# abargum/RAVE

Measured on AMD Instinct MI355X. Metric: audio samples/sec/GPU (48 kHz v2 encode+decode); × real-time factor, higher is better.
Workload: dtype fp32 (per conv / fused unit the faster of exact-fp32 MFMA and fp32 on the bf16 matrix cores: operands split exactly into 3 bf16 parts (24 significand bits), 6 of the 9 cross products (the 3 dropped are each < 2^-25 |a b|), fp32 accumulate; edges exact-fp32 MFMA); 1 GPU; v2 non-causal encode+decode, 16 x 65536 samples per GPU (BASELINE configs[1]); global_batch=16, samples_per_clip=65536, parallelism=dp1 (batch shards, RCCL all-gather of latents)

## Files before the change

### include/rave_amd.h

```cpp
#ifndef RAVE_AMD_H
#define RAVE_AMD_H

#include <stddef.h>
#include <stdint.h>

#ifdef __cplusplus
extern "C" {
#endif

#define RAVE_ABI_VERSION 21
#define RAVE_SPLITK_TICKETS 4096
#define RAVE_SPLITK_STATUS_WORD (RAVE_SPLITK_TICKETS - 1)

enum {
    RAVE_OK = 0,
    RAVE_ERR_ARG = -1,
    RAVE_ERR_HIP = -2,
    RAVE_ERR_UNSUPPORTED = -3,
    RAVE_ERR_STATE = -4,
    RAVE_ERR_COOP = -5
};

enum { RAVE_ACT_NONE = 0, RAVE_ACT_LEAKY = 1, RAVE_ACT_SNAKE = 2 };

// ... 169 lines not shown
    int32_t batch, frames, n_band, noise_bands;
    int32_t target, _pad0;
    const float* amp; int64_t a_sb, a_sc;
    const float* u;   int64_t u_sb;
    const float* gy;  int64_t gy_sb, gy_sc;
    float* gamp;      int64_t ga_sb, ga_sc;
} rave_noise_backward_args;
int rave_noise_synth_backward(const rave_noise_backward_args* a, void* stream);

typedef struct rave_adain_args {
    int32_t batch, channels, t_len, mode;
    int32_t max_batch, row0;
    const float* x; int64_t x_sb, x_sc;
    float* y;       int64_t y_sb, y_sc;
    float* stats;
    float* counters;
    uint32_t* ticket;
} rave_adain_args;
int rave_adain(const rave_adain_args* a, void* stream);

typedef struct rave_adain_backward_args {
    int32_t batch, channels, t_len, mode;
    int32_t max_batch, row0;
    const float* gy; int64_t gy_sb, gy_sc;
    float* gx;       int64_t gx_sb, gx_sc;
    const float* stats;
    const float* counters;
} rave_adain_backward_args;
int rave_adain_backward(const rave_adain_backward_args* a, void* stream);

typedef struct rave_unit_args {
    int32_t channels, batch, t_len, dilation;
    int32_t pad_left, act;
    float leaky_slope; int32_t precision;
    const float* x; int64_t x_sb, x_sc;
    float* y;       int64_t y_sb, y_sc;
    const float* weight;
    const float* bias1; const float* bias2;
    const float* alpha0; const float* alpha2;
    float* workspace;
    uint32_t* status;
    int32_t x_len;
    int32_t res_shift;
    int32_t coop_rb;
    int32_t reserved0;
} rave_unit_args;
int64_t rave_unit_packed_size(int channels);
int rave_unit_pack_weight(const float* w1, const float* w2, int channels, float* packed);
int64_t rave_unit_split_packed_size(int channels);
int rave_unit_split_pack_weight(const float* w1, const float* w2, int channels, float* packed);
int rave_unit_ring_pack_weight(const float* w1, const float* w2, int channels, float* packed);
int64_t rave_unit_bf3_packed_size(int channels);
int rave_unit_bf3_pack_weight(const float* w1, const float* w2, int channels, float* packed);
int64_t rave_unit_workspace(const rave_unit_args* a);
int rave_residual_unit(const rave_unit_args* a, void* stream);
int rave_debug_coop(int64_t spin_limit, int force_giveup);

#define RAVE_STACK_UNITS 3
typedef struct rave_stack_args {
    int32_t channels, batch, t_len, act;
    float leaky_slope; int32_t precision;
    int32_t dilation[RAVE_STACK_UNITS], pad_left[RAVE_STACK_UNITS];
    const float* x; int64_t x_sb, x_sc;
    float* y;       int64_t y_sb, y_sc;
    const float* weight[RAVE_STACK_UNITS];
    const float* bias1[RAVE_STACK_UNITS];
    const float* bias2[RAVE_STACK_UNITS];
    const float* alpha0[RAVE_STACK_UNITS];
    const float* alpha2[RAVE_STACK_UNITS];
} rave_stack_args;
int rave_stack_supported(int channels);
int rave_residual_stack(const rave_stack_args* a, void* stream);

typedef struct rave_edge_args {
    int32_t batch, frames;
    int32_t conv_c_in, conv_c_out, conv_kernel, conv_pad_left;
    int32_t pqmf_taps, pqmf_pad_left;
    int32_t mode, act;
    float leaky_slope;
    int32_t fill_channels, fill_t;
    int32_t precision;
    const float* x;     int64_t x_sb, x_sc;
    float* y;           int64_t y_sb, y_sc;
    const float* weight;
    const float* bias;
    const float* alpha;
    const float* filter;
    const float* noise; int64_t n_sb, n_sc;
    float* fill_y;      int64_t f_sb, f_sc;
    const float* fill_values;
    int64_t fill_vs;
} rave_edge_args;
int rave_encoder_head(const rave_edge_args* a, void* stream);
int rave_decoder_tail(const rave_edge_args* a, void* stream);
#define RAVE_EDGE_FILTER_FLOATS 8836
int rave_encoder_head_pack_filter(const float* hkf, int n_band, int taps, int n_out_bands, float* image);
int rave_decoder_tail_pack_filter(const float* hki, int n_band, int taps, float* image);
int rave_encoder_head_pack_filter_f32(const float* hkf, int n_band, int taps, int n_out_bands, float* image);
int rave_decoder_tail_pack_filter_f32(const float* hki, int n_band, int taps, float* image);

enum {
    RAVE_OP_CONV = 1,
    RAVE_OP_PQMF_ANALYSIS = 2,
    RAVE_OP_PQMF_SYNTHESIS = 3,
    RAVE_OP_FILL = 4,
    RAVE_OP_RVQ_ENCODE = 5,
// ... 265 lines not shown
```

### rave_amd/_native.py

```python
from __future__ import annotations

import ctypes as C
import os

_HERE = os.path.dirname(os.path.abspath(__file__))
LIB_PATH = os.path.join(_HERE, "librave_amd.so")
if os.environ.get("RAVE_AMD_DIAG_LIB") == "1":
    LIB_PATH = os.path.join(_HERE, "librave_amd_diag.so")
if os.environ.get("RAVE_AMD_LIB_VARIANT"):
    LIB_PATH = os.path.join(_HERE, f"librave_amd_{os.environ['RAVE_AMD_LIB_VARIANT']}.so")

RAVE_OK = 0
RAVE_ERR_ARG = -1
RAVE_ERR_HIP = -2
RAVE_ERR_UNSUPPORTED = -3
RAVE_ERR_STATE = -4
RAVE_ERR_COOP = -5

ACT = {"none": 0, "leaky": 1, "snake": 2}

OP_CONV = 1
OP_PQMF_ANALYSIS = 2
OP_PQMF_SYNTHESIS = 3
OP_FILL = 4
# ... 253 lines not shown
class ModelConfig(C.Structure):
    _fields_ = [("n_band", i32), ("enc_bands", i32), ("capacity", i32), ("latent_size", i32),
                ("kernel_size", i32), ("speaker_size", i32), ("n_ratios", i32),
                ("ratios", i32 * MAX_RATIOS), ("n_dilations", i32 * MAX_RATIOS),
                ("dilations", (i32 * MAX_DILATIONS) * MAX_RATIOS),
                ("amplitude_modulation", i32), ("causal", i32), ("activation", i32), ("adain", i32),
                ("leaky_slope", f32), ("conv_bias", i32), ("convt_bias", i32),
                ("noise", i32), ("noise_hidden", i32), ("noise_bands", i32), ("n_noise_ratios", i32),
                ("noise_ratios", i32 * MAX_RATIOS), ("rvq_quantizers", i32), ("rvq_codebook_size", i32),
                ("fuse_units", i32), ("speaker_rows", i32)]


class Param(C.Structure):
    _fields_ = [("name", C.c_char_p), ("data", vp), ("numel", i64)]


class OpInfo(C.Structure):
    _fields_ = [("kind", i32), ("precision", i32), ("flops", C.c_double), ("bytes", C.c_double),
                ("label", C.c_char * 96)]


PAYLOAD = 240


class PlanOp(C.Structure):
    _fields_ = [("kind", i32), ("_pad0", i32), ("raw", C.c_ubyte * PAYLOAD)]


class Reloc(C.Structure):
    _fields_ = [("op", i32), ("field_offset", i32), ("slot", i32), ("_pad0", i32),
                ("byte_offset", i64)]


STRUCTS = [ConvArgs, AnalysisArgs, SynthesisArgs, FillArgs, RvqArgs, ShiftArgs, PlanOp, Reloc,
           CopyArgs, NoiseArgs, AdainArgs, UnitArgs, StackArgs, ModelConfig, Param, OpInfo,
           FirArgs, RowStatsArgs, AttnPoolArgs, LinearArgs, MaxPoolArgs, EdgeArgs,
           StftArgs, DistanceArgs, YinArgs, F0OneHotArgs, SynthesisBackwardArgs, AnalysisBackwardArgs,
           ConvBackwardArgs, NoiseBackwardArgs, AdainBackwardArgs, StftLossArgs]

EXPORTS = [
    "rave_last_error", "rave_abi_version", "rave_struct_sizes",
    "rave_conv1d_chunk", "rave_conv1d_packed_size", "rave_conv1d_pack_weight", "rave_conv1d_pack_weight_device",
    "rave_conv1d",
    "rave_conv1d_workspace", "rave_conv1d_backward_workspace", "rave_conv1d_backward_data",
    "rave_conv1d_backward_weight", "rave_conv_transpose1d_backward_workspace", "rave_conv_transpose1d_backward_data",
    "rave_conv_transpose1d_backward_weight", "rave_conv1d_configs", "rave_conv1d_split_packed_size", "rave_conv1d_split_pack_weight",
    "rave_conv1d_ring_pack_weight", "rave_conv1d_bf3_packed_size", "rave_conv1d_bf3_pack_weight",
    "rave_pqmf_analysis", "rave_pqmf_synthesis", "rave_pqmf_analysis_backward", "rave_pqmf_synthesis_backward",
    "rave_fill_channels", "rave_copy",
    "rave_rvq_workspace", "rave_rvq_encode", "rave_rvq_decode", "rave_shift_history", "rave_noise_synth", "rave_adain",
    "rave_noise_synth_backward", "rave_adain_backward",
    "rave_unit_packed_size", "rave_unit_pack_weight", "rave_residual_unit",
    "rave_unit_split_packed_size", "rave_unit_split_pack_weight", "rave_unit_ring_pack_weight",
    "rave_unit_bf3_packed_size", "rave_unit_bf3_pack_weight",
    "rave_unit_workspace", "rave_debug_coop", "rave_model_check",
    "rave_stack_supported", "rave_residual_stack",
    "rave_plan_create", "rave_plan_run", "rave_plan_destroy", "rave_plan_size",
    "rave_plan_profile", "rave_plan_op_times", "rave_fill_uniform",
    "rave_model_param_count", "rave_model_param_info", "rave_model_create", "rave_model_destroy",
    "rave_model_encode", "rave_model_decode", "rave_model_forward", "rave_model_encode_codes",
    "rave_model_decode_codes", "rave_model_noise_shape", "rave_model_adain_control", "rave_model_set_row0",
    "rave_model_set_speaker", "rave_model_set_speakers", "rave_model_set_speaker_row0", "rave_model_speaker_info",
    "rave_model_adain_count", "rave_model_adain_info", "rave_model_adain_get", "rave_model_adain_set",
    "rave_model_tuning_get", "rave_model_tuning_set", "rave_model_plan_ops", "rave_model_profile",
    "rave_model_op_times", "rave_stream_create", "rave_stream_destroy", "rave_stream_reset",
    "rave_stream_encode", "rave_stream_decode", "rave_stream_encode_codes", "rave_stream_decode_codes",
    "rave_stream_delay",
    "rave_stream_launches",
    "rave_fir", "rave_row_stats", "rave_attn_pool", "rave_linear", "rave_maxpool",
    "rave_encoder_head", "rave_decoder_tail", "rave_encoder_head_pack_filter", "rave_decoder_tail_pack_filter",
    "rave_encoder_head_pack_filter_f32", "rave_decoder_tail_pack_filter_f32",
    "rave_stft_table_size", "rave_stft_pack_table", "rave_stft_mag",
    "rave_audio_distance_workspace", "rave_audio_distance",
    "rave_yin_shape", "rave_yin", "rave_f0_onehot", "rave_pitch_onehot",
    "rave_stft_loss_table_size", "rave_stft_loss_pack_table", "rave_stft_loss_workspace",
    "rave_stft_loss_forward", "rave_stft_loss_backward",
]
EDGE_FILTER_FLOATS = 8836


class NativeError(RuntimeError):
    pass


def _load():
    if not os.path.exists(LIB_PATH):
        raise ImportError(f"rave_amd native library not built: {LIB_PATH} is missing "
                          "(run `python -c 'import __graft_entry__ as g; g.build()'` or "
                          "`make -C rave_amd/csrc`)")
    lib = C.CDLL(LIB_PATH)
    lib.rave_last_error.restype = C.c_char_p
    lib.rave_abi_version.restype = C.c_int
    lib.rave_struct_sizes.argtypes = [C.POINTER(i64), C.c_int]
    lib.rave_conv1d_chunk.argtypes = [C.c_int] * 5
    lib.rave_conv1d_packed_size.argtypes = [C.c_int] * 6
    lib.rave_conv1d_packed_size.restype = i64
    lib.rave_conv1d_pack_weight.argtypes = [vp] + [C.c_int] * 7 + [vp]
    lib.rave_conv1d_pack_weight_device.argtypes = [vp] + [C.c_int] * 7 + [vp, vp]
    lib.rave_conv1d_workspace.argtypes = [C.POINTER(ConvArgs)]
    lib.rave_conv1d_configs.argtypes = [C.POINTER(ConvArgs), C.POINTER(i32), C.c_int]
    lib.rave_conv1d_split_packed_size.argtypes = [C.c_int] * 6
    lib.rave_conv1d_split_packed_size.restype = i64
    lib.rave_conv1d_split_pack_weight.argtypes = [vp] + [C.c_int] * 7 + [vp]
    lib.rave_conv1d_ring_pack_weight.argtypes = [vp] + [C.c_int] * 7 + [vp]
    lib.rave_conv1d_bf3_packed_size.argtypes = [C.c_int] * 6
    lib.rave_conv1d_bf3_packed_size.restype = i64
    lib.rave_conv1d_bf3_pack_weight.argtypes = [vp] + [C.c_int] * 7 + [vp]
    lib.rave_encoder_head_pack_filter.argtypes = [vp, C.c_int, C.c_int, C.c_int, vp]
    lib.rave_encoder_head_pack_filter_f32.argtypes = [vp, C.c_int, C.c_int, C.c_int, vp]
    lib.rave_decoder_tail_pack_filter_f32.argtypes = [vp, C.c_int, C.c_int, vp]
    lib.rave_decoder_tail_pack_filter.argtypes = [vp, C.c_int, C.c_int, vp]
    lib.rave_unit_packed_size.argtypes = [C.c_int]
    lib.rave_unit_packed_size.restype = i64
    lib.rave_unit_pack_weight.argtypes = [vp, vp, C.c_int, vp]
    lib.rave_unit_workspace.argtypes = [C.c_void_p]
    lib.rave_unit_workspace.restype = i64
    lib.rave_debug_coop.argtypes = [i64, C.c_int]
    lib.rave_unit_split_packed_size.argtypes = [C.c_int]
    lib.rave_stack_supported.argtypes = [C.c_int]
    lib.rave_unit_split_packed_size.restype = i64
    lib.rave_unit_split_pack_weight.argtypes = [vp, vp, C.c_int, vp]
    lib.rave_unit_ring_pack_weight.argtypes = [vp, vp, C.c_int, vp]
    lib.rave_unit_bf3_packed_size.argtypes = [C.c_int]
    lib.rave_unit_bf3_packed_size.restype = i64
    lib.rave_unit_bf3_pack_weight.argtypes = [vp, vp, C.c_int, vp]
    lib.rave_conv1d_workspace.restype = i64
    lib.rave_conv1d_backward_workspace.argtypes = [C.POINTER(ConvBackwardArgs)]
    lib.rave_conv1d_backward_workspace.restype = i64
    lib.rave_conv_transpose1d_backward_workspace.argtypes = [C.POINTER(ConvBackwardArgs)]
    lib.rave_conv_transpose1d_backward_workspace.restype = i64
    lib.rave_rvq_workspace.argtypes = [C.POINTER(RvqArgs)]
    lib.rave_rvq_workspace.restype = i64
    for name, st in [("rave_conv1d", ConvArgs), ("rave_pqmf_analysis", AnalysisArgs),
                     ("rave_pqmf_synthesis", SynthesisArgs), ("rave_fill_channels", FillArgs),
                     ("rave_pqmf_synthesis_backward", SynthesisBackwardArgs),
                     ("rave_pqmf_analysis_backward", AnalysisBackwardArgs),
                     ("rave_conv1d_backward_data", ConvBackwardArgs),
                     ("rave_conv1d_backward_weight", ConvBackwardArgs),
                     ("rave_conv_transpose1d_backward_data", ConvBackwardArgs),
                     ("rave_conv_transpose1d_backward_weight", ConvBackwardArgs),
                     ("rave_rvq_encode", RvqArgs), ("rave_rvq_decode", RvqArgs),
                     ("rave_shift_history", ShiftArgs), ("rave_copy", CopyArgs),
                     ("rave_noise_synth", NoiseArgs), ("rave_adain", AdainArgs),
                     ("rave_noise_synth_backward", NoiseBackwardArgs), ("rave_adain_backward", AdainBackwardArgs),
                     ("rave_residual_unit", UnitArgs), ("rave_residual_stack", StackArgs),
                     ("rave_fir", FirArgs), ("rave_row_stats", RowStatsArgs), ("rave_attn_pool", AttnPoolArgs),
                     ("rave_linear", LinearArgs), ("rave_maxpool", MaxPoolArgs),
                     ("rave_encoder_head", EdgeArgs), ("rave_decoder_tail", EdgeArgs)]:
        getattr(lib, name).argtypes = [C.POINTER(st), vp]
    lib.rave_stft_table_size.argtypes = [C.c_int]
    lib.rave_stft_table_size.restype = i64
    lib.rave_stft_pack_table.argtypes = [C.c_int, vp]
    lib.rave_stft_mag.argtypes = [C.POINTER(StftArgs), vp]
    lib.rave_audio_distance_workspace.argtypes = [C.POINTER(DistanceArgs)]
    lib.rave_audio_distance_workspace.restype = i64
    lib.rave_audio_distance.argtypes = [C.POINTER(DistanceArgs), vp]
    lib.rave_stft_loss_table_size.argtypes = [C.c_int, C.c_int]
    lib.rave_stft_loss_table_size.restype = i64
    lib.rave_stft_loss_pack_table.argtypes = [C.c_int, C.c_int, vp]
    lib.rave_stft_loss_workspace.argtypes = [C.POINTER(StftLossArgs)]
    lib.rave_stft_loss_workspace.restype = i64
    lib.rave_stft_loss_forward.argtypes = [C.POINTER(StftLossArgs), vp]
    lib.rave_stft_loss_backward.argtypes = [C.POINTER(StftLossArgs), vp]
    lib.rave_yin_shape.argtypes = [C.POINTER(YinArgs), C.POINTER(i32)]
    lib.rave_yin.argtypes = [C.POINTER(YinArgs), vp]
    lib.rave_f0_onehot.argtypes = [C.POINTER(F0OneHotArgs), vp]
    lib.rave_pitch_onehot.argtypes = [C.POINTER(YinArgs), C.POINTER(F0OneHotArgs), vp]
    lib.rave_plan_create.argtypes = [C.POINTER(PlanOp), C.c_int, C.POINTER(Reloc), C.c_int,
                                     C.POINTER(vp)]
    lib.rave_plan_run.argtypes = [vp, C.POINTER(vp), C.c_int, vp]
    lib.rave_plan_destroy.argtypes = [vp]
    lib.rave_plan_size.argtypes = [vp]
    lib.rave_plan_profile.argtypes = [vp, C.c_int]
    lib.rave_plan_op_times.argtypes = [vp, C.POINTER(C.c_float), C.c_int]
    lib.rave_fill_uniform.argtypes = [vp, i64, C.c_uint64, f32, f32, vp]
    cfgp = C.POINTER(ModelConfig)
    lib.rave_model_param_count.argtypes = [cfgp]
    lib.rave_model_param_info.argtypes = [cfgp, C.c_int, C.c_char_p, C.c_int, C.POINTER(i64)]
# ... 205 lines not shown
```

### rave_amd/csrc/unit_split.hip

```cpp
#include "common.h"
#include "pack_shared.h"

#include <algorithm>
#include <atomic>
#include <cmath>
#include <cstdlib>
#include <cstring>
#include <vector>

namespace rave {

typedef _Float16 us_h8 __attribute__((ext_vector_type(8)));
typedef _Float16 us_h4 __attribute__((ext_vector_type(4)));
typedef float us_f32x8 __attribute__((ext_vector_type(8)));
typedef float us_f32x4 __attribute__((ext_vector_type(4)));
typedef float us_f32x16 __attribute__((ext_vector_type(16)));
typedef unsigned us_u32x4 __attribute__((ext_vector_type(4)));
typedef __bf16 us_b8 __attribute__((ext_vector_type(8)));
typedef __bf16 us_b4 __attribute__((ext_vector_type(4)));

constexpr int kUSMaxDil = 16;
#ifndef RAVE_US_R
#define RAVE_US_R 3
#endif
// ... 13 lines not shown
#define US_AT(k, kc)                               \
    do {                                           \
        if ((k) >= 0) RAVE_STAMP(g_us_stamps, k); \
    } while (0)
#endif
constexpr unsigned kUSOOB = 0xFFFFFFF0u;
constexpr int kXcds = 8;
constexpr int kCoopNoFit = 1;
constexpr int kCoopMaxRB = 4;

struct USArgs {
    const float* x; float* y; const float* w; const float* rs1; const float* rs2;
    const float* b1; const float* b2; const float* a0; const float* a2;
    int64_t x_sb, x_sc, y_sb, y_sc;
    int T, d, pad_l, ntiles, XW;
    int XL, rsh;
    int x_bytes, y_bytes, w_bytes, bias_bytes;
    int act;
    float slope;
    unsigned xw_magic;
    unsigned* flags; unsigned* tmo; float* xmax; float* xch;
    int ngroups, xch_bytes;
    int xv;
    unsigned nb_magic;
    int flag_stride;
    unsigned* status;
    unsigned spin_limit;
    int force_giveup;
};

constexpr int kUSBf512Dil = 4;
template <int C, int WGN, int MI, int KG = 1, int CB = 2, int RB = 1, int NP = 2> struct USGeo {
    static constexpr int WGM = C / (32 * MI * RB), NWT = WGM * WGN, NW = NWT * KG, NT = 64 * NW;
    static constexpr int BN = 32 * CB * WGN;
    static constexpr int S1 = 3 * C / 16, S2 = C / 16, ST = S1 + S2;
    static constexpr int PH = C + 8;
    static constexpr int XW_MAX = BN + 2 * ((NP == 3 && C == 512) ? kUSBf512Dil : kUSMaxDil);
    static constexpr int XPLANE = XW_MAX * PH * 2;
    static constexpr int HPLANE = BN * PH * 2;
    static constexpr int PL1 = XPLANE > HPLANE ? XPLANE : HPLANE;
    static constexpr int PLANES = NP * PL1;
    static constexpr int TAB = PLANES, VOTE = PLANES + 6 * C * 4, VRED = VOTE + 16;
    static constexpr int LDS = VRED + 64;
    static constexpr int G8 = C / 8;
    static constexpr int XT = (XW_MAX * G8 + NT - 1) / NT;
    static constexpr int R = RB > 1 ? RAVE_US_RC : RAVE_US_R;
    static constexpr int G8R = C / (8 * RB);
    static constexpr int RED = NWT * MI * CB * 16 * 64 * 4;
    static_assert(C % 64 == 0 && (MI == 1 || MI == 2) && NW <= 16, "geometry");
    static_assert(RB == 1 || (KG == 1 && WGN == 1 && C % (32 * MI * RB) == 0), "cooperative geometry");
    static_assert(KG == 1 || (KG == 2 && S1 % 2 == 0 && S2 % 2 == 0 && RED <= PLANES), "K-groups");
};

template <int C, int WGN, int MI, int KG, int CB, bool SNAKE, int AR, int RB, bool GUARD>
__device__ __forceinline__ bool unit_split_body(const USArgs& a) {
    constexpr bool F32 = AR == 1, BF = AR == 2;
    constexpr int NPW = BF ? 3 : 2;
    using G = USGeo<C, WGN, MI, KG, CB, RB, NPW>;
    constexpr bool SC1X = RB > 1 && 2 * G::LDS > 160 * 1024;
    static_assert(!SC1X || 2 * G::LDS > 160 * 1024, "sc1 hand-off: one workgroup per CU only");
    constexpr bool GV = GUARD && AR == 0;
    static_assert(RB == 1 || GUARD || AR != 0, "the cooperative split16 form runs guarded");
    constexpr int NT = G::NT, PH = G::PH, G8 = G::G8, XT = G::XT, R = G::R;
    constexpr int S1 = G::S1, ST = G::ST, CG = C / 16;
    extern __shared__ __attribute__((aligned(16))) char lds[];
    _Float16* ph = reinterpret_cast<_Float16*>(lds);
    _Float16* pl = reinterpret_cast<_Float16*>(lds + G::PL1);
    _Float16* pm = reinterpret_cast<_Float16*>(lds + 2 * G::PL1);
    float* pf = reinterpret_cast<float*>(lds);
    float* tab = reinterpret_cast<float*>(lds + G::TAB);
    unsigned char* vote = reinterpret_cast<unsigned char*>(lds + G::VOTE);
    float* vred = reinterpret_cast<float*>(lds + G::VRED);

    US_AT(0, 0);
    const int tid = threadIdx.x;
    const int lane = tid & 63;
    const int wave = __builtin_amdgcn_readfirstlane(tid >> 6);
    const int kg = wave / G::NWT;
    const int twave = wave - kg * G::NWT;
    const int wm = twave % G::WGM, wn = twave / G::WGM;
    const int hh = lane >> 5, l32 = lane & 31;
    int lg, rb = 0;
    if constexpr (RB == 1) {
        lg = __builtin_amdgcn_readfirstlane(xcd_major(blockIdx.x, gridDim.x));
    } else {
        const int q = blockIdx.x >> 3;
        rb = q % RB;
        lg = (blockIdx.x & 7) * (int)(gridDim.x / (8 * RB)) + q / RB;
        if (lg >= a.ngroups) return true;
    }
    const int b = lg / a.ntiles;
    const int n0 = (lg - b * a.ntiles) * G::BN;
    const float slope = a.act == RAVE_ACT_LEAKY ? a.slope : 1.0f;
    const int XW = a.XW;
    const int ntask = XW * G8;
    const int t0 = n0 - a.pad_l;

    const auto xrs = make_rsrc(a.x + (int64_t)b * a.x_sb, a.x_bytes);
    const auto wrs = make_rsrc(a.w, a.w_bytes);
    int sh0 = 0, sh2 = 0;

    us_h8 ring[R][MI][NPW];
    const int wmg = wm + rb * G::WGM;
    const unsigned abase = (unsigned)((MI * wmg) * ST * NPW) * 1024u + (unsigned)lane * 16u;
    auto load_a = [&](int slot, int s) __attribute__((always_inline)) {
#pragma unroll
        for (int i = 0; i < MI; ++i)
#pragma unroll
            for (int p = 0; p < NPW; ++p)
                ring[slot][i][p] = __builtin_bit_cast(us_h8, __builtin_amdgcn_raw_buffer_load_b128(
                    wrs, s < ST ? abase + (unsigned)(((i * ST + s) * NPW + p) * 1024) : kUSOOB, 0, 0));
    };
    auto prefetch_ring = [&]() __attribute__((always_inline)) {
#pragma unroll
        for (int t = 0; t < R; ++t) load_a(t, t * KG + kg);
    };
    if (!a.xv) prefetch_ring();

    constexpr int NTAB = (6 * C + NT - 1) / NT;
    float tabv[NTAB];
#pragma unroll
    for (int r = 0; r < NTAB; ++r) {
        const int i = tid + r * NT;
        const int k = __builtin_amdgcn_readfirstlane(i / C), m = i - k * C;
        const float* src = k == 0 ? a.rs1 : k == 1 ? a.b1 : k == 2 ? a.a2 : k == 3 ? a.rs2 : k == 4 ? a.b2 : a.a0;
        const bool has = k < 6 && ((k == 1 || k == 4) ? a.bias_bytes > 0 : (k == 2 || k == 5) ? SNAKE : true);
        tabv[r] = has ? src[m] : 0.f;
    }
    auto store_tab = [&]() __attribute__((always_inline)) {
#pragma unroll
        for (int r = 0; r < NTAB; ++r)
            if (__builtin_amdgcn_readfirstlane(tid + r * NT) < 6 * C) tab[tid + r * NT] = tabv[r];
    };

    auto stage_window = [&](float xs) __attribute__((always_inline)) {
        float cmax = 0.f;
        float rx[XT][8];
#pragma unroll
        for (int i = 0; i < XT; ++i) {
            const int e = tid + i * NT;
            const int g = (int)(((unsigned)e * a.xw_magic) >> 24);
            const int w = e - g * XW;
            const int t = min(max(t0 + w, 0), a.XL - 1);
#pragma unroll
            for (int v = 0; v < 8; ++v) {
                const int c = min(g * 8 + v, C - 1);
                rx[i][v] = __builtin_bit_cast(float, __builtin_amdgcn_raw_buffer_load_b32(
                    xrs, (unsigned)(c * a.x_sc + t) * 4u, 0, 0));
            }
        }
#pragma unroll
        for (int i = 0; i < XT; ++i) {
            const int e = tid + i * NT;
            const int g = (int)(((unsigned)e * a.xw_magic) >> 24);
            const int w = e - g * XW;
            const bool ok = (e < ntask) && (t0 + w >= 0) && (t0 + w < a.XL);
            us_f32x8 v8;
#pragma unroll
            for (int v = 0; v < 8; ++v) {
                const float al = SNAKE ? a.a0[min(g * 8 + v, C - 1)] : 0.f;
                v8[v] = ok ? act<SNAKE>(rx[i][v], slope, al) * xs : 0.f;
            }
            if constexpr (F32) {
                if (e < ntask) {
                    *reinterpret_cast<us_f32x4*>(pf + w * PH + g * 8) = us_f32x4{v8[0], v8[1], v8[2], v8[3]};
                    *reinterpret_cast<us_f32x4*>(pf + w * PH + g * 8 + 4) = us_f32x4{v8[4], v8[5], v8[6], v8[7]};
                }
            } else if constexpr (BF) {
                us_b8 hi, mid, lo;
                bf3_split_pk(v8, hi, mid, lo);
// ... 28 lines not shown
            const int kb = e - g * nb;
            const int t = ta + 4 * kb;
            const bool ok = (e < ntv) && t >= 0 && t < a.XL;
#pragma unroll
            for (int v = 0; v < 8; ++v) {
                rx[i][v] = __builtin_bit_cast(us_f32x4, __builtin_amdgcn_raw_buffer_load_b128(
                    xrs, ok ? (unsigned)((g * 8 + v) * a.x_sc + t) * 4u : kUSOOB, 0, 0));
            }
        }
        prefetch_ring();
        if constexpr (SNAKE) {
            store_tab();
            __syncthreads();
        }
        if (RB == 1) US_AT(6, -1);
#pragma unroll
        for (int i = 0; i < XTV; ++i) {
            const int e = tid + i * NT;
            const int g = (int)(((unsigned)e * a.nb_magic) >> 24);
            const int kb = e - g * nb;
            if (e < ntv) {
                float al[8];
#pragma unroll
                for (int v = 0; v < 8; ++v) al[v] = SNAKE ? tab[5 * C + g * 8 + v] : 0.f;
#pragma unroll
                for (int q = 0; q < 4; ++q) {
                    const int w = ta + 4 * kb + q - t0;
                    us_f32x8 v8;
#pragma unroll
                    for (int v = 0; v < 8; ++v) v8[v] = act<SNAKE>(rx[i][v][q], slope, al[v]);
                    if (w < 0 || w >= XW) continue;
                    if constexpr (F32) {
                        *reinterpret_cast<us_f32x4*>(pf + w * PH + g * 8) = us_f32x4{v8[0], v8[1], v8[2], v8[3]};
                        *reinterpret_cast<us_f32x4*>(pf + w * PH + g * 8 + 4) = us_f32x4{v8[4], v8[5], v8[6], v8[7]};
                    } else if constexpr (BF) {
                        us_b8 hi, mid, lo;
                        bf3_split_pk(v8, hi, mid, lo);
                        *reinterpret_cast<us_b8*>(ph + w * PH + g * 8) = hi;
                        *reinterpret_cast<us_b8*>(pl + w * PH + g * 8) = lo;
                        *reinterpret_cast<us_b8*>(pm + w * PH + g * 8) = mid;
                    } else {
                        cmax = fmaxf(cmax, absmax8(v8));
                        const us_h8 hi = __builtin_convertvector(v8, us_h8);
                        const us_h8 lo = __builtin_convertvector((v8 - __builtin_convertvector(hi, us_f32x8)) * 2048.0f, us_h8);
                        *reinterpret_cast<us_h8*>(ph + w * PH + g * 8) = hi;
                        *reinterpret_cast<us_h8*>(pl + w * PH + g * 8) = lo;
                    }
                }
            }
        }
        if constexpr (!SNAKE) store_tab();
        return cmax;
    };
    {
        float cmax;
        if (a.xv) {
            cmax = stage_window_v();
        } else {
            store_tab();
            cmax = stage_window(1.0f);
        }
        if constexpr (GV) vote_cast(vote, wave, cmax);
        __syncthreads();
        if (GV && __builtin_expect(vote_any<G::NW>(vote), 0)) {
            sh0 = __builtin_amdgcn_readfirstlane(split_shift(block_max<G::NW>(cmax, vred)));
            const float xs = ldexpf(1.0f, -sh0);
#pragma nounroll
            for (int e = tid; e < ntask; e += NT) {
                const int g = (int)(((unsigned)e * a.xw_magic) >> 24);
                const int w = e - g * XW;
                const bool ok = (t0 + w >= 0) && (t0 + w < a.XL);
                const int t = min(max(t0 + w, 0), a.XL - 1);
                us_f32x8 v8;
#pragma unroll
                for (int v = 0; v < 8; ++v) {
                    const int c = min(g * 8 + v, C - 1);
                    const float xv = __builtin_bit_cast(float, __builtin_amdgcn_raw_buffer_load_b32(
                        xrs, (unsigned)(c * a.x_sc + t) * 4u, 0, 0));
                    v8[v] = ok ? act<SNAKE>(xv, slope, SNAKE ? a.a0[c] : 0.f) * xs : 0.f;
                }
                const us_h8 hi = __builtin_convertvector(v8, us_h8);
                const us_h8 lo = __builtin_convertvector((v8 - __builtin_convertvector(hi, us_f32x8)) * 2048.0f, us_h8);
                *reinterpret_cast<us_h8*>(ph + w * PH + g * 8) = hi;
                *reinterpret_cast<us_h8*>(pl + w * PH + g * 8) = lo;
            }
            __syncthreads();
        }
    }
    US_AT(1, 1);

    constexpr bool DA = RB > 1;
    us_f32x16 acc[MI][CB], accb[MI][CB];
    auto zero_acc = [&]() __attribute__((always_inline)) {
#pragma unroll
        for (int i = 0; i < MI; ++i)
#pragma unroll
            for (int j = 0; j < CB; ++j)
#pragma unroll
                for (int r = 0; r < 16; ++r) acc[i][j][r] = accb[i][j][r] = 0.f;
    };
    auto fold_acc = [&]() __attribute__((always_inline)) {
        if constexpr (DA) {
#pragma unroll
            for (int i = 0; i < MI; ++i)
#pragma unroll
                for (int j = 0; j < CB; ++j) acc[i][j] += accb[i][j];
        }
    };
    zero_acc();

    const int col0 = wn * 32 * CB + l32;
    struct BFr {
        us_h8 h[CB], l[CB], m[CB];
    };
    auto read_b = [&](int s, BFr& f) __attribute__((always_inline)) {
        int row, ch;
        if (s < S1) {
            const int tap = s / CG;
            row = col0 + tap * a.d;
            ch = (s - tap * CG) * 16;
        } else {
            row = col0;
            ch = (s - S1) * 16;
        }
#pragma unroll
        for (int j = 0; j < CB; ++j) {
            const int off = (row + j * 32) * PH + ch + 8 * hh;
            if constexpr (F32) {
                f.h[j] = *reinterpret_cast<const us_h8*>(pf + off);
                f.l[j] = *reinterpret_cast<const us_h8*>(pf + off + 4);
            } else {
                f.h[j] = *reinterpret_cast<const us_h8*>(ph + off);
                f.l[j] = *reinterpret_cast<const us_h8*>(pl + off);
                if constexpr (BF) f.m[j] = *reinterpret_cast<const us_h8*>(pm + off);
            }
        }
    };
    auto smap = [&](int t) __attribute__((always_inline)) {
        if (RB == 1 || t < S1 || t >= ST) return t;
        int u = t - S1 + rb * (CG / RB);
        if (u >= CG) u -= CG;
        return S1 + u;
    };
    auto step = [&](int t, int s, const BFr& f, us_f32x16 (&acc)[MI][CB]) __attribute__((always_inline)) {
        us_h8 ah[MI], al[MI], a2[MI];
#pragma unroll
        for (int i = 0; i < MI; ++i) {
            ah[i] = ring[t % R][i][0];
            al[i] = ring[t % R][i][1];
            a2[i] = ah[i] * (_Float16)2048.0f;
        }
        if constexpr (BF) {
            us_b8 wh[MI], wl[MI], wmd[MI];
#pragma unroll
            for (int i = 0; i < MI; ++i) {
                wh[i] = __builtin_bit_cast(us_b8, ring[t % R][i][0]);
                wl[i] = __builtin_bit_cast(us_b8, ring[t % R][i][1]);
                wmd[i] = __builtin_bit_cast(us_b8, ring[t % R][i][2]);
            }
            load_a(t % R, RB > 1 ? smap(t + R) : s + R * KG);
#pragma unroll
            for (int i = 0; i < MI; ++i)
#pragma unroll
                for (int j = 0; j < CB; ++j) {
                    const us_b8 xh = __builtin_bit_cast(us_b8, f.h[j]), xl = __builtin_bit_cast(us_b8, f.l[j]),
                                xm = __builtin_bit_cast(us_b8, f.m[j]);
                    acc[i][j] = __builtin_amdgcn_mfma_f32_32x32x16_bf16(wl[i], xh, acc[i][j], 0, 0, 0);
                    acc[i][j] = __builtin_amdgcn_mfma_f32_32x32x16_bf16(wh[i], xl, acc[i][j], 0, 0, 0);
                    acc[i][j] = __builtin_amdgcn_mfma_f32_32x32x16_bf16(wmd[i], xm, acc[i][j], 0, 0, 0);
                    acc[i][j] = __builtin_amdgcn_mfma_f32_32x32x16_bf16(wmd[i], xh, acc[i][j], 0, 0, 0);
                    acc[i][j] = __builtin_amdgcn_mfma_f32_32x32x16_bf16(wh[i], xm, acc[i][j], 0, 0, 0);
                    acc[i][j] = __builtin_amdgcn_mfma_f32_32x32x16_bf16(wh[i], xh, acc[i][j], 0, 0, 0);
                }
            return;
        }
        load_a(t % R, RB > 1 ? smap(t + R) : s + R * KG);
        if constexpr (F32) {
#pragma unroll
            for (int hf = 0; hf < 2; ++hf)
#pragma unroll
                for (int e = 0; e < 4; ++e)
#pragma unroll
                    for (int i = 0; i < MI; ++i)
#pragma unroll
                        for (int j = 0; j < CB; ++j) {
                            const us_f32x4 wv = __builtin_bit_cast(us_f32x4, hf ? al[i] : ah[i]);
                            const us_f32x4 xv = __builtin_bit_cast(us_f32x4, hf ? f.l[j] : f.h[j]);
                            acc[i][j] = __builtin_amdgcn_mfma_f32_32x32x2f32(wv[e], xv[e], acc[i][j], 0, 0, 0);
                        }
            return;
        }
#pragma unroll
        for (int i = 0; i < MI; ++i)
#pragma unroll
            for (int j = 0; j < CB; ++j) acc[i][j] = __builtin_amdgcn_mfma_f32_32x32x16_f16(a2[i], f.h[j], acc[i][j], 0, 0, 0);
#pragma unroll
        for (int i = 0; i < MI; ++i)
#pragma unroll
            for (int j = 0; j < CB; ++j) acc[i][j] = __builtin_amdgcn_mfma_f32_32x32x16_f16(ah[i], f.l[j], acc[i][j], 0, 0, 0);
#pragma unroll
        for (int i = 0; i < MI; ++i)
#pragma unroll
            for (int j = 0; j < CB; ++j) acc[i][j] = __builtin_amdgcn_mfma_f32_32x32x16_f16(al[i], f.h[j], acc[i][j], 0, 0, 0);
    };

    const int mrow0 = 32 * MI * wmg + 4 * hh;
    auto kloop = [&](auto gtag, auto t0tag, auto t1tag) __attribute__((always_inline)) {
        constexpr int GG = decltype(gtag)::value;
        constexpr int T0 = decltype(t0tag)::value, T1 = decltype(t1tag)::value;
        BFr f[2];
        auto sidx = [&](int t) __attribute__((always_inline)) { return RB > 1 ? smap(t) : t * KG + GG; };
        read_b(sidx(T0), f[0]);
#pragma unroll
        for (int t = T0; t < T1; ++t) {
            if (t + 1 < T1) read_b(sidx(t + 1), f[(t + 1 - T0) & 1]);
            __builtin_amdgcn_sched_barrier(0);
            if (DA && ((t - T0) & 1)) step(t, sidx(t), f[(t - T0) & 1], accb);
            else step(t, sidx(t), f[(t - T0) & 1], acc);
        }
    };
    float* red = reinterpret_cast<float*>(lds);
    auto combine = [&]() __attribute__((always_inline)) {
        if constexpr (KG == 2) {
            __syncthreads();
            float* mine = red + twave * (MI * CB * 16 * 64);
            if (kg == 1) {
#pragma unroll
                for (int i = 0; i < MI; ++i)
#pragma unroll
                    for (int j = 0; j < CB; ++j)
#pragma unroll
                        for (int r = 0; r < 16; ++r) mine[((i * CB + j) * 16 + r) * 64 + lane] = acc[i][j][r];
            }
            __syncthreads();
            if (kg == 0) {
#pragma unroll
                for (int i = 0; i < MI; ++i)
#pragma unroll
                    for (int j = 0; j < CB; ++j)
#pragma unroll
                        for (int r = 0; r < 16; ++r) acc[i][j][r] += mine[((i * CB + j) * 16 + r) * 64 + lane];
            }
        }
    };
    if (KG == 1 || kg == 0) kloop(IC<0>{}, IC<0>{}, IC<S1 / KG>{});
    else kloop(IC<1>{}, IC<0>{}, IC<S1 / KG>{});
    fold_acc();
    combine();
    __syncthreads();
    US_AT(2, 2);

    const float f0 = ldexpf(1.0f, sh0);
    const auto xcrs = make_rsrc(a.xch, RB > 1 ? a.xch_bytes : 0);
    const unsigned xslot = (unsigned)lg * (unsigned)(G::BN * C);
    auto seam = [&](float xs, auto pubtag) __attribute__((always_inline)) {
        constexpr bool publish = decltype(pubtag)::value != 0 && RB > 1;
        float cmax = 0.f;
        if (KG == 1 || kg == 0) {
#pragma unroll
            for (int i = 0; i < MI; ++i)
#pragma unroll
                for (int g = 0; g < 4; ++g) {
                    const int m = mrow0 + 32 * i + 8 * g;
                    const us_f32x4 rs = *reinterpret_cast<const us_f32x4*>(tab + m) * f0;
                    const us_f32x4 bb = *reinterpret_cast<const us_f32x4*>(tab + C + m);
                    us_f32x4 al = {0.f, 0.f, 0.f, 0.f};
                    if constexpr (SNAKE) al = *reinterpret_cast<const us_f32x4*>(tab + 2 * C + m);
#pragma unroll
                    for (int j = 0; j < CB; ++j) {
                        us_f32x4 v;
#pragma unroll
                        for (int e = 0; e < 4; ++e)
                            v[e] = act<SNAKE>(acc[i][j][4 * g + e] * rs[e] + bb[e], slope, al[e]) * xs;
                        if constexpr (publish)
                            __builtin_amdgcn_raw_buffer_store_b128(
                                __builtin_bit_cast(us_u32x4, v), xcrs,
                                (xslot + (unsigned)((col0 + 32 * j) * C + m)) * 4u, 0, 16);
                        if constexpr (F32) {
                            *reinterpret_cast<us_f32x4*>(pf + (col0 + 32 * j) * PH + m) = v;
                            continue;
                        }
                        if constexpr (BF) {
                            us_b4 hi, mid, lo;
                            bf3_split_pk(v, hi, mid, lo);
                            *reinterpret_cast<us_b4*>(ph + (col0 + 32 * j) * PH + m) = hi;
                            *reinterpret_cast<us_b4*>(pl + (col0 + 32 * j) * PH + m) = lo;
                            *reinterpret_cast<us_b4*>(pm + (col0 + 32 * j) * PH + m) = mid;
                            continue;
                        }
#pragma unroll
                        for (int e = 0; e < 4; ++e) cmax = fmaxf(cmax, fabsf(v[e]));
                        const us_h4 hv = __builtin_convertvector(v, us_h4);
                        const us_h4 lv = __builtin_convertvector((v - __builtin_convertvector(hv, us_f32x4)) * 2048.0f, us_h4);
                        *reinterpret_cast<us_h4*>(ph + (col0 + 32 * j) * PH + m) = hv;
                        *reinterpret_cast<us_h4*>(pl + (col0 + 32 * j) * PH + m) = lv;
                    }
                }
        }
        return cmax;
// ... 177 lines not shown
            const int n = n0 + col0 + 32 * j;
            const bool nok = n < a.T;
#pragma unroll
            for (int i = 0; i < MI; ++i)
#pragma unroll
                for (int r = 0; r < 16; ++r) {
                    const int m = mrow0 + 32 * i + 8 * (r >> 2) + (r & 3);
                    res[i][j][r] = __builtin_bit_cast(float, __builtin_amdgcn_raw_buffer_load_b32(
                        xrs, nok ? (unsigned)(m * a.x_sc + n + a.rsh) * 4u : kUSOOB, 0, 0));
                }
        }
#pragma unroll
        for (int i = 0; i < MI; ++i)
#pragma unroll
            for (int g = 0; g < 4; ++g) {
                const int m = mrow0 + 32 * i + 8 * g;
                const us_f32x4 rs = *reinterpret_cast<const us_f32x4*>(tab + 3 * C + m) * f2;
                const us_f32x4 bb = *reinterpret_cast<const us_f32x4*>(tab + 4 * C + m);
#pragma unroll
                for (int j = 0; j < CB; ++j) {
                    const int n = n0 + col0 + 32 * j;
                    const bool nok = n < a.T;
#pragma unroll
                    for (int e = 0; e < 4; ++e)
                        __builtin_amdgcn_raw_buffer_store_b32(
                            __builtin_bit_cast(unsigned, gave_up ? __builtin_nanf("")
                                                                 : acc[i][j][4 * g + e] * rs[e] + bb[e] + res[i][j][4 * g + e]),
                            yrs, nok ? (unsigned)((m + e) * a.y_sc + n) * 4u : kUSOOB, 0, 0);
                }
            }
    }
    US_AT(5, -1);
    if constexpr (CHECK && KG == 1) {
        if (vote_rerun()) return false;
    }
    return true;
}

template <int C, int WGN, int MI, int KG, int CB, bool SNAKE, int RB>
__global__ __launch_bounds__(64 * (C / (32 * MI * RB)) * WGN * KG) void unit_split_kernel(USArgs a) {
    if constexpr (RB > 1) {
        (void)unit_split_body<C, WGN, MI, KG, CB, SNAKE, 0, RB, true>(a);
    } else {
        if (!unit_split_body<C, WGN, MI, KG, CB, SNAKE, 0, RB, false>(a))
            (void)unit_split_body<C, WGN, MI, KG, CB, SNAKE, 0, RB, true>(a);
    }
}
template <int C, int WGN, int MI, int KG, int CB, bool SNAKE, int RB>
__global__ __launch_bounds__(64 * (C / (32 * MI * RB)) * WGN * KG) void unit_ring_f32_kernel(USArgs a) {
    (void)unit_split_body<C, WGN, MI, KG, CB, SNAKE, 1, RB, false>(a);
}
template <int C, int WGN, int MI, int KG, int CB, bool SNAKE, int RB>
__global__ __launch_bounds__(64 * (C / (32 * MI * RB)) * WGN * KG) void unit_bf3_kernel(USArgs a) {
    (void)unit_split_body<C, WGN, MI, KG, CB, SNAKE, 2, RB, false>(a);
}

static int coop_max_queues() {
    static const int q = [] {
        const char* e = std::getenv("GPU_MAX_HW_QUEUES");
        const int v = e ? std::atoi(e) : 0;
        return v > 0 ? v : 4;
    }();
    return q;
}

template <int C, int WGN, int MI, int KG, int CB, int RB = 1>
static int us_launch(USArgs k, int B, bool snake, int ar, hipStream_t st) {
    using G = USGeo<C, WGN, MI, KG, CB, RB>;
    using G3 = USGeo<C, WGN, MI, KG, CB, RB, 3>;
    const bool f32 = ar == 1;
    if (k.XW > (ar == 2 ? G3::XW_MAX : G::XW_MAX)) {
        set_error(ar == 2 && C == 512 ? "residual_unit(bf16x3): C = 512 supports dilations <= 4"
                                      : "residual_unit(split16): dilation too large");
        return RAVE_ERR_UNSUPPORTED;
    }
    k.ntiles = ceil_div(k.T, G::BN);
    void (*kern)(USArgs) = nullptr;
    int lds = G::LDS;
    if (ar == 2) {
        if constexpr (G3::LDS <= 160 * 1024) {
            kern = snake ? unit_bf3_kernel<C, WGN, MI, KG, CB, true, RB> : unit_bf3_kernel<C, WGN, MI, KG, CB, false, RB>;
            lds = G3::LDS;
        } else {
            set_error("residual_unit(bf16x3): this width does not fit the CU's LDS as three planes");
            return RAVE_ERR_UNSUPPORTED;
        }
    } else {
        kern = f32 ? (snake ? unit_ring_f32_kernel<C, WGN, MI, KG, CB, true, RB> : unit_ring_f32_kernel<C, WGN, MI, KG, CB, false, RB>)
                   : (snake ? unit_split_kernel<C, WGN, MI, KG, CB, true, RB> : unit_split_kernel<C, WGN, MI, KG, CB, false, RB>);
    }
    static bool attr[6] = {false, false, false, false, false, false};
    if (lds > 65536 && !attr[2 * ar + snake]) {
        RAVE_CHECK_HIP(hipFuncSetAttribute(reinterpret_cast<const void*>(kern),
                                           hipFuncAttributeMaxDynamicSharedMemorySize, lds));
        attr[2 * ar + snake] = true;
    }
    int grid = k.ntiles * B;
    if constexpr (RB > 1) {
        static int fits[6] = {-1, -1, -1, -1, -1, -1};
        int& f = fits[2 * ar + snake];
        if (f < 0) {
            int per_cu = 0, dev = 0, cus = 0;
            RAVE_CHECK_HIP(hipOccupancyMaxActiveBlocksPerMultiprocessor(&per_cu, reinterpret_cast<const void*>(kern),
                                                                        G::NT, lds));
            RAVE_CHECK_HIP(hipGetDevice(&dev));
            RAVE_CHECK_HIP(hipDeviceGetAttribute(&cus, hipDeviceAttributeMultiprocessorCount, dev));
            const int64_t q = coop_max_queues();
// ... 21 lines not shown
extern "C" int64_t rave_unit_split_packed_size(int C) { return unit_packed_floats(C, 2); }
extern "C" int64_t rave_unit_bf3_packed_size(int C) { return unit_packed_floats(C, 3); }

static int unit_pack(const float* w1, const float* w2, int C, float* packed, int mode) {
    const bool f32 = mode != kPackSplit16;
    RAVE_CHECK_ARG(w1 && w2 && packed, "unit_split_pack_weight: null pointer");
    if (!us_supported(C)) {
        set_error("unit_split_pack_weight: split16 fused residual unit supports C in {64, 128, 256, 512}");
        return RAVE_ERR_UNSUPPORTED;
    }
    const int S1 = 3 * C / 16, ST = 4 * C / 16, CG = C / 16;
    std::vector<int> e1(C), e2(C);
    for (int m = 0; m < C; ++m) {
        double a1 = 0.0, a2 = 0.0;
        for (int k = 0; k < 3 * C; ++k) a1 = std::max(a1, (double)std::fabs(w1[(int64_t)m * 3 * C + k]));
        for (int k = 0; k < C; ++k) a2 = std::max(a2, (double)std::fabs(w2[(int64_t)m * C + k]));
        e1[m] = f32 ? 0 : row_exponent(a1);
        e2[m] = f32 ? 0 : row_exponent(a2);
    }
    for (int mb = 0; mb < C / 32; ++mb)
        for (int s = 0; s < ST; ++s)
            for (int l = 0; l < 64; ++l)
                for (int e = 0; e < 8; ++e) {
                    const int m = mb * 32 + (l & 31);
                    const int kk = 8 * (l >> 5) + e;
                    float v;
                    if (s < S1) {
                        const int tap = s / CG, ci = (s % CG) * 16 + kk;
                        v = std::ldexp(w1[((int64_t)m * C + ci) * 3 + tap], e1[m]);
                    } else {
                        const int ci = (s - S1) * 16 + kk;
                        v = std::ldexp(w2[(int64_t)m * C + ci], e2[m]);
                    }
                    put_fragment(packed, (int64_t)mb * ST + s, mode, l, e, v);
                }
    float* rs = packed + packed_floats((int64_t)(C / 32) * ST, pack_planes(mode), 0);
    for (int m = 0; m < C; ++m) {
        rs[m] = f32 ? 1.0f : (float)std::ldexp(1.0, -(e1[m] + 11));
        rs[C + m] = f32 ? 1.0f : (float)std::ldexp(1.0, -(e2[m] + 11));
    }
    return RAVE_OK;
}

extern "C" int rave_unit_split_pack_weight(const float* w1, const float* w2, int C, float* packed) {
    return unit_pack(w1, w2, C, packed, kPackSplit16);
}

extern "C" int rave_unit_ring_pack_weight(const float* w1, const float* w2, int C, float* packed) {
    return unit_pack(w1, w2, C, packed, kPackF32);
}

extern "C" int rave_unit_bf3_pack_weight(const float* w1, const float* w2, int C, float* packed) {
    return unit_pack(w1, w2, C, packed, kPackBf16x3);
}

#ifdef RAVE_STAMPS
extern "C" int rave_diag_unit_stamps(void* p) {
    RAVE_CHECK_HIP(hipMemcpyToSymbol(HIP_SYMBOL(g_us_stamps), &p, sizeof(p)));
    return RAVE_OK;
}
#endif

namespace rave {
static std::atomic<unsigned> g_coop_spin{kUSSpinLimit};
static std::atomic<int> g_coop_force{0};
static bool coop_enabled() {
    static const bool on = [] {
        const char* e = std::getenv("RAVE_UNIT_COOP");
        return !(e && e[0] == '0');
    }();
    return on;
}
constexpr int kCoopBN = 32;
struct CoopLayout {
    int rb = 1, stride = 2;
    int64_t groups = 0, xmax = 0, xch = 0, floats = 0;
};
static CoopLayout coop_layout(const rave_unit_args& a) {
    CoopLayout L;
    const int C = a.channels;
    if ((C != 256 && C != 512) || !coop_enabled() || a.batch <= 0 || a.t_len <= 0) return L;
    if (a.precision != RAVE_PREC_SPLIT16 && a.precision != RAVE_PREC_F32_RING && a.precision != RAVE_PREC_BF16X3)
        return L;
    const int64_t ng = (int64_t)ceil_div(a.t_len, kCoopBN) * a.batch;
    const int64_t ngp = ceil_div64(ng, 8) * 8;
    if (2 * ngp > RAVE_SPLITK_STATUS_WORD) return L;
    while (L.stride < 32 && 2 * L.stride * ngp <= RAVE_SPLITK_STATUS_WORD) L.stride *= 2;
    const int rb = a.coop_rb == 4 && C == 256 ? 4 : C / 128;
    if (a.coop_rb != 0 && a.coop_rb != rb) return L;
    L.groups = ng;
    L.xmax = RAVE_SPLITK_TICKETS;
    L.xch = L.xmax + ceil_div64(ngp * rb, 64) * 64;
    L.floats = L.xch + ngp * kCoopBN * C;
    if (ngp * kCoopBN * C * 4 >= (1ll << 31)) return CoopLayout{};
    L.rb = rb;
    return L;
}

int residual_unit_split(const rave_unit_args& a, void* stream) {
    const int C = a.channels;
    if (!us_supported(C)) {
        set_error("residual_unit(split16): fused unit supports C in {64, 128, 256, 512}");
        return RAVE_ERR_UNSUPPORTED;
    }
    if (a.coop_rb != 0 && !((C == 256 && (a.coop_rb == 2 || a.coop_rb == 4)) || (C == 512 && a.coop_rb == 4))) {
        set_error("residual_unit: coop_rb must be 0, or 2 / 4 at C = 256, 4 at C = 512");
// ... 136 lines not shown
```

Before: 1.415 billion samples/s.

## Overlap bf16x3 window staging with first-conv MFMA steps via channel chunks

```diff
diff --git a/include/rave_amd.h b/include/rave_amd.h
--- a/include/rave_amd.h
+++ b/include/rave_amd.h
@@ -245,6 +245,7 @@
 int rave_unit_ring_pack_weight(const float* w1, const float* w2, int channels, float* packed);
 int64_t rave_unit_bf3_packed_size(int channels);
 int rave_unit_bf3_pack_weight(const float* w1, const float* w2, int channels, float* packed);
+int rave_unit_bf3_step_map(int channels, int coop_rb, int* steps, int cap);
 int64_t rave_unit_workspace(const rave_unit_args* a);
 int rave_residual_unit(const rave_unit_args* a, void* stream);
 int rave_debug_coop(int64_t spin_limit, int force_giveup);
diff --git a/rave_amd/_native.py b/rave_amd/_native.py
--- a/rave_amd/_native.py
+++ b/rave_amd/_native.py
@@ -329,7 +329,7 @@
     "rave_noise_synth_backward", "rave_adain_backward",
     "rave_unit_packed_size", "rave_unit_pack_weight", "rave_residual_unit",
     "rave_unit_split_packed_size", "rave_unit_split_pack_weight", "rave_unit_ring_pack_weight",
-    "rave_unit_bf3_packed_size", "rave_unit_bf3_pack_weight",
+    "rave_unit_bf3_packed_size", "rave_unit_bf3_pack_weight", "rave_unit_bf3_step_map",
     "rave_unit_workspace", "rave_debug_coop", "rave_model_check",
     "rave_stack_supported", "rave_residual_stack",
     "rave_plan_create", "rave_plan_run", "rave_plan_destroy", "rave_plan_size",
@@ -401,6 +401,7 @@
     lib.rave_unit_bf3_packed_size.argtypes = [C.c_int]
     lib.rave_unit_bf3_packed_size.restype = i64
     lib.rave_unit_bf3_pack_weight.argtypes = [vp, vp, C.c_int, vp]
+    lib.rave_unit_bf3_step_map.argtypes = [C.c_int, C.c_int, C.POINTER(i32), C.c_int]
     lib.rave_conv1d_workspace.restype = i64
     lib.rave_conv1d_backward_workspace.argtypes = [C.POINTER(ConvBackwardArgs)]
     lib.rave_conv1d_backward_workspace.restype = i64
diff --git a/rave_amd/csrc/unit_split.hip b/rave_amd/csrc/unit_split.hip
--- a/rave_amd/csrc/unit_split.hip
+++ b/rave_amd/csrc/unit_split.hip
@@ -89,9 +89,30 @@
     static_assert(KG == 1 || (KG == 2 && S1 % 2 == 0 && S2 % 2 == 0 && RED <= PLANES), "K-groups");
 };
 
-template <int C, int WGN, int MI, int KG, int CB, bool SNAKE, int AR, int RB, bool GUARD>
+constexpr int us_chunk_step(int C, int NCH, int t) {
+    const int CG = C / 16, CGC = CG / NCH, SC = 3 * CGC;
+    const int c = t / SC, u = t - c * SC, tap = u / CGC;
+    return tap * CG + c * CGC + (u - tap * CGC);
+}
+constexpr bool us_chunk_map_ok(int C, int NCH) {
+    const int CG = C / 16, S1 = 3 * CG;
+    if (NCH < 1 || CG % NCH != 0 || S1 > 96) return false;
+    bool seen[96] = {};
+    for (int t = 0; t < S1; ++t) {
+        const int s = us_chunk_step(C, NCH, t);
+        if (s < 0 || s >= S1 || seen[s]) return false;
+        seen[s] = true;
+        if ((s % CG) * 16 + 16 > (t / (S1 / NCH) + 1) * (C / NCH)) return false;
+    }
+    return true;
+}
+constexpr int us_bf3_chunks(int C, int RB) { return RB > 1 ? 2 : 1; }
+
+template <int C, int WGN, int MI, int KG, int CB, bool SNAKE, int AR, int RB, bool GUARD, int NCH = 1>
 __device__ __forceinline__ bool unit_split_body(const USArgs& a) {
     constexpr bool F32 = AR == 1, BF = AR == 2;
+    static_assert(NCH == 1 || (BF && us_chunk_map_ok(C, NCH) && (3 * C / 16) % (NCH * KG) == 0),
+                  "window chunks: bf16x3 only, whole 16-channel groups and K-group steps per chunk");
     constexpr int NPW = BF ? 3 : 2;
     using G = USGeo<C, WGN, MI, KG, CB, RB, NPW>;
     constexpr bool SC1X = RB > 1 && 2 * G::LDS > 160 * 1024;
@@ -152,7 +173,7 @@
 #pragma unroll
         for (int t = 0; t < R; ++t) load_a(t, t * KG + kg);
     };
-    if (!a.xv) prefetch_ring();
+    if (NCH == 1 && !a.xv) prefetch_ring();
 
     constexpr int NTAB = (6 * C + NT - 1) / NT;
     float tabv[NTAB];
@@ -287,7 +308,7 @@
         if constexpr (!SNAKE) store_tab();
         return cmax;
     };
-    {
+    if constexpr (NCH == 1) {
         float cmax;
         if (a.xv) {
             cmax = stage_window_v();
@@ -321,8 +342,8 @@
             }
             __syncthreads();
         }
-    }
-    US_AT(1, 1);
+        US_AT(1, 1);
+    }
 
     constexpr bool DA = RB > 1;
     us_f32x16 acc[MI][CB], accb[MI][CB];
@@ -372,12 +393,13 @@
         }
     };
     auto smap = [&](int t) __attribute__((always_inline)) {
+        if (NCH > 1 && t < S1) return us_chunk_step(C, NCH, t);
         if (RB == 1 || t < S1 || t >= ST) return t;
         int u = t - S1 + rb * (CG / RB);
         if (u >= CG) u -= CG;
         return S1 + u;
     };
-    auto step = [&](int t, int s, const BFr& f, us_f32x16 (&acc)[MI][CB]) __attribute__((always_inline)) {
+    auto step = [&](int t, int sn, const BFr& f, us_f32x16 (&acc)[MI][CB]) __attribute__((always_inline)) {
         us_h8 ah[MI], al[MI], a2[MI];
 #pragma unroll
         for (int i = 0; i < MI; ++i) {
@@ -393,7 +415,7 @@
                 wl[i] = __builtin_bit_cast(us_b8, ring[t % R][i][1]);
                 wmd[i] = __builtin_bit_cast(us_b8, ring[t % R][i][2]);
             }
-            load_a(t % R, RB > 1 ? smap(t + R) : s + R * KG);
+            load_a(t % R, sn);
 #pragma unroll
             for (int i = 0; i < MI; ++i)
 #pragma unroll
@@ -409,7 +431,7 @@
                 }
             return;
         }
-        load_a(t % R, RB > 1 ? smap(t + R) : s + R * KG);
+        load_a(t % R, sn);
         if constexpr (F32) {
 #pragma unroll
             for (int hf = 0; hf < 2; ++hf)
@@ -444,14 +466,14 @@
         constexpr int GG = decltype(gtag)::value;
         constexpr int T0 = decltype(t0tag)::value, T1 = decltype(t1tag)::value;
         BFr f[2];
-        auto sidx = [&](int t) __attribute__((always_inline)) { return RB > 1 ? smap(t) : t * KG + GG; };
+        auto sidx = [&](int t) __attribute__((always_inline)) { return smap(t * KG + GG); };
         read_b(sidx(T0), f[0]);
 #pragma unroll
         for (int t = T0; t < T1; ++t) {
             if (t + 1 < T1) read_b(sidx(t + 1), f[(t + 1 - T0) & 1]);
             __builtin_amdgcn_sched_barrier(0);
-            if (DA && ((t - T0) & 1)) step(t, sidx(t), f[(t - T0) & 1], accb);
-            else step(t, sidx(t), f[(t - T0) & 1], acc);
+            if (DA && ((t - T0) & 1)) step(t, sidx(t + R), f[(t - T0) & 1], accb);
+            else step(t, sidx(t + R), f[(t - T0) & 1], acc);
         }
     };
     float* red = reinterpret_cast<float*>(lds);
@@ -478,8 +500,112 @@
             }
         }
     };
-    if (KG == 1 || kg == 0) kloop(IC<0>{}, IC<0>{}, IC<S1 / KG>{});
-    else kloop(IC<1>{}, IC<0>{}, IC<S1 / KG>{});
+    auto phase1_chunked = [&](auto xvtag, auto gtag) __attribute__((always_inline)) {
+        constexpr bool XV = decltype(xvtag)::value != 0;
+        constexpr int GG = decltype(gtag)::value;
+        constexpr int G8C = G8 / NCH, SCL = S1 / (NCH * KG);
+        constexpr int NBM = (G::XW_MAX + 3) / 4 + 1;
+        constexpr int NTK = ((XV ? G8C * NBM : G8C * G::XW_MAX) + NT - 1) / NT;
+        constexpr int NU = XV ? 4 * NTK : NTK;
+        const int ta = t0 & ~3;
+        const int per = XV ? (t0 + XW - ta + 3) >> 2 : XW;
+        const unsigned magic = XV ? a.nb_magic : a.xw_magic;
+        const int ntc = G8C * per;
+        us_f32x4 rv[2][XV ? NTK : 1][8];
+        float rs[2][XV ? 1 : NTK][8];
+        auto sidx = [&](int t) __attribute__((always_inline)) { return smap(t * KG + GG); };
+        auto issue = [&](int c) __attribute__((always_inline)) {
+#pragma unroll
+            for (int i = 0; i < NTK; ++i) {
+                const int e = tid + i * NT;
+                const int gl = (int)(((unsigned)e * magic) >> 24);
+                const int k = e - gl * per;
+                const int g = c * G8C + gl;
+                if constexpr (XV) {
+                    const int t = ta + 4 * k;
+                    const bool ok = (e < ntc) && t >= 0 && t < a.XL;
+#pragma unroll
+                    for (int v = 0; v < 8; ++v)
+                        rv[c & 1][i][v] = __builtin_bit_cast(us_f32x4, __builtin_amdgcn_raw_buffer_load_b128(
+                            xrs, ok ? (unsigned)((g * 8 + v) * a.x_sc + t) * 4u : kUSOOB, 0, 0));
+                } else {
+                    const int t = min(max(t0 + k, 0), a.XL - 1);
+#pragma unroll
+                    for (int v = 0; v < 8; ++v)
+                        rs[c & 1][i][v] = __builtin_bit_cast(float, __builtin_amdgcn_raw_buffer_load_b32(
+                            xrs, (e < ntc) ? (unsigned)((g * 8 + v) * a.x_sc + t) * 4u : kUSOOB, 0, 0));
+                }
+            }
+        };
+        auto split_row = [&](int c, int u) __attribute__((always_inline)) {
+            const int i = XV ? u >> 2 : u, q = u & 3;
+            const int e = tid + i * NT;
+            const int gl = (int)(((unsigned)e * magic) >> 24);
+            const int k = e - gl * per;
+            const int g = c * G8C + gl;
+            const int w = XV ? ta + 4 * k + q - t0 : k;
+            const bool live = (e < ntc) && w >= 0 && w < XW;
+            const bool inx = XV || ((t0 + w >= 0) && (t0 + w < a.XL));
+            us_f32x8 v8;
+#pragma unroll
+            for (int v = 0; v < 8; ++v) {
+                const float al = SNAKE ? tab[5 * C + min(g, G8 - 1) * 8 + v] : 0.f;
+                const float xv = XV ? rv[c & 1][i][v][q] : rs[c & 1][i][v];
+                v8[v] = inx ? act<SNAKE>(xv, slope, al) : 0.f;
+            }
+            us_b8 hi, mid, lo;
+            bf3_split_pk(v8, hi, mid, lo);
+            if (live) {
+                *reinterpret_cast<us_b8*>(ph + w * PH + g * 8) = hi;
+                *reinterpret_cast<us_b8*>(pl + w * PH + g * 8) = lo;
+                *reinterpret_cast<us_b8*>(pm + w * PH + g * 8) = mid;
+            }
+        };
+        issue(0);
+#pragma unroll
+        for (int t = 0; t < R; ++t) load_a(t, sidx(t));
+        issue(1);
+        store_tab();
+        if constexpr (SNAKE) __syncthreads();
+        if (RB == 1) US_AT(6, -1);
+#pragma unroll
+        for (int u = 0; u < NU; ++u) split_row(0, u);
+        __syncthreads();
+        US_AT(1, 1);
+#pragma unroll
+        for (int c = 0; c < NCH; ++c) {
+            if (c + 2 < NCH) issue(c + 2);
+            BFr f[2];
+            const int T0 = c * SCL;
+            read_b(sidx(T0), f[0]);
+#pragma unroll
+            for (int tl = 0; tl < SCL; ++tl) {
+                const int t = T0 + tl;
+                if (tl + 1 < SCL) read_b(sidx(t + 1), f[(tl + 1) & 1]);
+                __builtin_amdgcn_sched_barrier(0);
+                if (DA && (tl & 1)) step(t, sidx(t + R), f[tl & 1], accb);
+                else step(t, sidx(t + R), f[tl & 1], acc);
+                if (c + 1 < NCH) {
+#pragma unroll
+                    for (int u = 0; u < NU; ++u)
+                        if (u * SCL / NU == tl) split_row(c + 1, u);
+                }
+            }
+            if (c + 1 < NCH) __syncthreads();
+        }
+    };
+    if constexpr (NCH > 1) {
+        if (KG == 1 || kg == 0) {
+            if (a.xv) phase1_chunked(IC<1>{}, IC<0>{});
+            else phase1_chunked(IC<0>{}, IC<0>{});
+        } else {
+            if (a.xv) phase1_chunked(IC<1>{}, IC<1>{});
+            else phase1_chunked(IC<0>{}, IC<1>{});
+        }
+    } else {
+        if (KG == 1 || kg == 0) kloop(IC<0>{}, IC<0>{}, IC<S1 / KG>{});
+        else kloop(IC<1>{}, IC<0>{}, IC<S1 / KG>{});
+    }
     fold_acc();
     combine();
     __syncthreads();
@@ -763,7 +889,7 @@
 }
 template <int C, int WGN, int MI, int KG, int CB, bool SNAKE, int RB>
 __global__ __launch_bounds__(64 * (C / (32 * MI * RB)) * WGN * KG) void unit_bf3_kernel(USArgs a) {
-    (void)unit_split_body<C, WGN, MI, KG, CB, SNAKE, 2, RB, false>(a);
+    (void)unit_split_body<C, WGN, MI, KG, CB, SNAKE, 2, RB, false, us_bf3_chunks(C, RB)>(a);
 }
 
 static int coop_max_queues() {
@@ -891,6 +1017,15 @@
 
 extern "C" int rave_unit_bf3_pack_weight(const float* w1, const float* w2, int C, float* packed) {
     return unit_pack(w1, w2, C, packed, kPackBf16x3);
+}
+
+extern "C" int rave_unit_bf3_step_map(int C, int coop_rb, int* steps, int cap) {
+    RAVE_CHECK_ARG(us_supported(C) && (coop_rb == 0 || coop_rb == 2 || coop_rb == 4), "unit_bf3_step_map: bad geometry");
+    const int S1 = 3 * C / 16;
+    RAVE_CHECK_ARG(steps && cap >= S1, "unit_bf3_step_map: steps[] holds fewer than 3 C / 16 entries");
+    const int nch = us_bf3_chunks(C, coop_rb ? coop_rb : 1);
+    for (int t = 0; t < S1; ++t) steps[t] = nch > 1 ? us_chunk_step(C, nch, t) : t;
+    return nch;
 }
 
 #ifdef RAVE_STAMPS
```

Result: no change. 1.418 billion samples/s, median of 6 (+0.2%).
